# StarRocks/starrocks

Hardware: AMD Instinct MI355X
Metric: ssb_join_agg_rows_per_sec (higher is better)
Workload: dtype int64; 1 GPU; ssb_sf100_q21_star_groupby; rows_per_gpu=600000000, seed=42, parallelism=dp1-replicated-dims

## Files before the change

### starrocks_amd/csrc/gpue.hip

```cpp
#include <hip/hip_runtime.h>
#include <cassert>
#include <cstdio>
#include <cstring>
#include <cstdlib>
#include <thread>
#include <algorithm>
#include <memory>
#include <type_traits>
#include <vector>
#include "gpue.h"

static thread_local char g_err[512] = {0};

const char* gpue_last_error(void) { return g_err; }

#define HIP_CHECK(expr)                                                      \
    do {                                                                     \
        hipError_t _e = (expr);                                              \
        if (_e != hipSuccess) {                                              \
            snprintf(g_err, sizeof(g_err), "%s failed: %s (%s:%d)", #expr,   \
                     hipGetErrorString(_e), __FILE__, __LINE__);             \
            return GPUE_ERR_HIP;                                             \
        }                                                                    \
    } while (0)

#define ARG_CHECK(cond)                                                      \
    do {                                                                     \
        if (!(cond)) {                                                       \
            snprintf(g_err, sizeof(g_err), "bad argument: %s (%s:%d)",       \
                     #cond, __FILE__, __LINE__);                             \
            return GPUE_ERR_ARG;                                             \
        }                                                                    \
    } while (0)

static constexpr int BLOCK = 256;
static constexpr int WAVE = 64;
static constexpr uint64_t MAX_GRID = 2048;

static uint32_t env_cap(const char* name, uint32_t dflt) {
    const char* e = getenv(name);
    int v = e ? atoi(e) : 0;
    return v > 0 ? (uint32_t)v : dflt;
}

static inline uint32_t grid_capped(uint64_t n, uint64_t cap) {
    uint64_t b = (n + BLOCK - 1) / BLOCK;
    if (b > cap) b = cap;
    if (b == 0) b = 1;
    return (uint32_t)b;
}

static inline uint32_t grid_for(uint64_t n) {
    static uint32_t cap = 0;
    if (!cap) cap = env_cap("GPUE_GRID", MAX_GRID);
    return grid_capped(n, cap);
}

static inline uint32_t grid_stream(uint64_t n) {
    static uint32_t cap = 0;
    if (!cap) cap = env_cap("GPUE_GRID_STREAM", 256);
    return grid_capped(n, cap);
}

__device__ static inline uint32_t join_mode_count(uint32_t c, int mode) {
    switch (mode) {
    case 1: return c ? 1u : 0u;
    case 2: return c ? 0u : 1u;
    case 3: return c ? c : 1u;
    default: return c;
    }
}

struct gpue_session {
    int device;
    hipStream_t stream;
    hipEvent_t ev_start, ev_stop;
    int32_t* d_datekey = nullptr;
    void* pinned = nullptr;
    static constexpr uint64_t PINNED_BYTES = 65536;
    hipStream_t stream2 = nullptr;
    static constexpr int N_CHUNK_EVENTS = 32;
    hipEvent_t chunk_ev[N_CHUNK_EVENTS] = {};
    unsigned int* d_agg_err = nullptr;
};
#define AGG_ERR_SENTINEL 1u
#define AGG_ERR_FULL 2u

struct gpue_dbuf {
    gpue_session* s;
    void* ptr;
    uint64_t bytes;
    bool owned = true;
};

struct gpue_join_table {
    gpue_session* s = nullptr;
    int64_t min_key = 0, max_key = 0;
    uint32_t* first = nullptr;
    uint32_t* next = nullptr;
    uint32_t* bitset = nullptr;
    int64_t set_min = 0, set_max = -1;
    uint16_t* first16 = nullptr;
    uint32_t* prefilter = nullptr;
    uint32_t* prefilter2w = nullptr;
    uint32_t* prefilter2 = nullptr;
    uint2* dense_groups = nullptr;
    uint64_t bucket_size = 0;
    uint64_t row_count = 0;
    enum Kind { PAYLOAD = 0, RANGE_DIRECT = 1, BUCKET_CHAINED = 2,
                DENSE_RANGE_DIRECT = 7, BUCKET_CHAINED128 = 8,
                LINEAR_CHAINED = 3, VARCHAR = 4, BUCKET_CHAINED64 = 5 } kind = PAYLOAD;
    uint32_t log_bucket_size = 0;
    uint32_t* build_keys = nullptr;
    uint8_t* key_bytes = nullptr;
    uint32_t* key_offsets = nullptr;
    uint8_t* key_nulls = nullptr;
    uint64_t* build_keys64 = nullptr;
    ulonglong2* build_keys128 = nullptr;
};

struct JoinTableDeleter {
    void operator()(gpue_join_table* t) const { gpue_join_table_destroy(t); }
};
using JoinTableOwner = std::unique_ptr<gpue_join_table, JoinTableDeleter>;

int gpue_device_count(int* out) {
    int n = 0;
    hipError_t e = hipGetDeviceCount(&n);
    if (e != hipSuccess) n = 0;
    *out = n;
    return GPUE_OK;
}

int gpue_session_create(int device_index, gpue_session** out) {
    ARG_CHECK(out != nullptr);
    int n = 0;
    if (hipGetDeviceCount(&n) != hipSuccess || n == 0) {
        snprintf(g_err, sizeof(g_err), "no AMD GPU visible (hipGetDeviceCount)");
        return GPUE_ERR_NO_GPU;
    }
    ARG_CHECK(device_index >= 0 && device_index < n);
    HIP_CHECK(hipSetDevice(device_index));
    gpue_session* s = new gpue_session();
    s->device = device_index;
    HIP_CHECK(hipStreamCreate(&s->stream));
    HIP_CHECK(hipEventCreate(&s->ev_start));
    HIP_CHECK(hipEventCreate(&s->ev_stop));
    HIP_CHECK(hipHostMalloc(&s->pinned, gpue_session::PINNED_BYTES));
    HIP_CHECK(hipStreamCreate(&s->stream2));
    for (int i = 0; i < gpue_session::N_CHUNK_EVENTS; i++)
        HIP_CHECK(hipEventCreateWithFlags(&s->chunk_ev[i], hipEventDisableTiming));
    HIP_CHECK(hipMalloc(&s->d_agg_err, sizeof(unsigned int)));
    HIP_CHECK(hipMemset(s->d_agg_err, 0, sizeof(unsigned int)));
    *out = s;
    return GPUE_OK;
}

static int agg_err_check(gpue_session* s, const char* what) {
    unsigned int e = 0;
    HIP_CHECK(hipMemcpy(&e, s->d_agg_err, sizeof(e), hipMemcpyDeviceToHost));
    if (e == 0) return GPUE_OK;
    HIP_CHECK(hipMemset(s->d_agg_err, 0, sizeof(e)));
    snprintf(g_err, sizeof(g_err), "%s: %s%s%s", what,
             (e & AGG_ERR_SENTINEL) ? "group key 0xFFFFFFFFFFFFFFFF collides with the "
                                      "empty-slot sentinel" : "",
             (e & (AGG_ERR_SENTINEL | AGG_ERR_FULL)) == (AGG_ERR_SENTINEL | AGG_ERR_FULL)
                 ? "; " : "",
             (e & AGG_ERR_FULL) ? "hash table full (capacity < distinct keys)" : "");
    return GPUE_ERR_ARG;
}

void gpue_session_destroy(gpue_session* s) {
    if (!s) return;
    if (s->d_agg_err) (void)hipFree(s->d_agg_err);
    if (s->pinned) (void)hipHostFree(s->pinned);
    for (int i = 0; i < gpue_session::N_CHUNK_EVENTS; i++)
        if (s->chunk_ev[i]) (void)hipEventDestroy(s->chunk_ev[i]);
    if (s->stream2) (void)hipStreamDestroy(s->stream2);
    if (s->d_datekey) (void)hipFree(s->d_datekey);
    (void)hipEventDestroy(s->ev_start);
    (void)hipEventDestroy(s->ev_stop);
    (void)hipStreamDestroy(s->stream);
    delete s;
}

// ... 1203 lines not shown
            hi = max(hi, (int32_t)i);
        }
    }
    for (int off = WAVE / 2; off > 0; off >>= 1) {
        lo = min(lo, __shfl_down(lo, off, WAVE));
        hi = max(hi, __shfl_down(hi, off, WAVE));
    }
    if ((threadIdx.x & (WAVE - 1)) == 0) {
        atomicMin(lo_out, lo);
        atomicMax(hi_out, hi);
    }
}

__global__ void k_build_prefilter_split_w(const uint32_t* __restrict__ bitset,
                                          uint64_t set_interval,
                                          uint32_t* __restrict__ pf2) {
    const uint32_t M19 = (1u << 19) - 1;
    uint64_t stride = (uint64_t)gridDim.x * blockDim.x;
    for (uint64_t i = (uint64_t)blockIdx.x * blockDim.x + threadIdx.x; i < set_interval;
         i += stride) {
        if ((bitset[i >> 5] >> (i & 31)) & 1u) {
            uint32_t a = (uint32_t)i & M19;
            uint32_t b = ((uint32_t)i * 2654435761u) >> 13;
            atomicOr(&pf2[a >> 5], 1u << (a & 31));
            atomicOr(&pf2[(1u << 14) + (b >> 5)], 1u << (b & 31));
        }
    }
}

__global__ void k_build_prefilter_split(const uint32_t* __restrict__ bitset,
                                        uint64_t set_interval,
                                        uint32_t* __restrict__ pf2) {
    const uint32_t M18 = (1u << 18) - 1;
    uint64_t stride = (uint64_t)gridDim.x * blockDim.x;
    for (uint64_t i = (uint64_t)blockIdx.x * blockDim.x + threadIdx.x; i < set_interval;
         i += stride) {
        if ((bitset[i >> 5] >> (i & 31)) & 1u) {
            uint32_t a = (uint32_t)i & M18;
            uint32_t b = ((uint32_t)i * 2654435761u) >> 14;
            atomicOr(&pf2[a >> 5], 1u << (a & 31));
            atomicOr(&pf2[(1u << 13) + (b >> 5)], 1u << (b & 31));
        }
    }
}

__global__ void k_build_prefilter(const uint32_t* __restrict__ bitset, uint64_t set_interval,
                                  uint32_t* __restrict__ prefilter) {
    uint64_t stride = (uint64_t)gridDim.x * blockDim.x;
    for (uint64_t i = (uint64_t)blockIdx.x * blockDim.x + threadIdx.x; i < set_interval;
         i += stride) {
        if ((bitset[i >> 5] >> (i & 31)) & 1u) {
            uint32_t f = (uint32_t)i & ((1u << 19) - 1);
            atomicOr(&prefilter[f >> 5], 1u << (f & 31));
        }
    }
}

__global__ void k_derive_bitset(const uint32_t* __restrict__ first, uint64_t offset,
                                uint64_t interval, uint32_t* __restrict__ bitset) {
    uint64_t nwords = (interval + 31) / 32;
    uint64_t stride = (uint64_t)gridDim.x * blockDim.x;
    for (uint64_t w = (uint64_t)blockIdx.x * blockDim.x + threadIdx.x; w < nwords; w += stride) {
        uint32_t bits = 0;
        uint64_t base = w * 32;
        #pragma unroll 4
        for (int j = 0; j < 32; j++) {
            uint64_t idx = base + j;
            if (idx < interval && first[offset + idx] != 0) bits |= (1u << j);
        }
        bitset[w] = bits;
    }
}

__global__ void k_derive_u16(const uint32_t* __restrict__ first, uint64_t interval,
                             uint16_t* __restrict__ first16, uint32_t* __restrict__ overflow) {
    uint64_t stride = (uint64_t)gridDim.x * blockDim.x;
    for (uint64_t i = (uint64_t)blockIdx.x * blockDim.x + threadIdx.x; i < interval; i += stride) {
        uint32_t v = first[i];
        if (v >= 65536u) atomicOr(overflow, 1u);
        first16[i] = (uint16_t)v;
    }
}

__global__ void k_build_range_direct(const int32_t* __restrict__ keys, uint64_t row_count,
                                     int64_t min_key, uint32_t* __restrict__ first,
                                     uint32_t* __restrict__ next) {
    uint64_t stride = (uint64_t)gridDim.x * blockDim.x;
    for (uint64_t i = 1 + (uint64_t)blockIdx.x * blockDim.x + threadIdx.x; i <= row_count;
         i += stride)
        next[i] = atomicExch(&first[keys[i] - min_key], (uint32_t)i);
}

static int join_table_minmax(gpue_session* s, const int32_t* d_keys, uint64_t n,
                             int64_t* mn_out, int64_t* mx_out) {
    int32_t h_init[2] = {INT32_MAX, INT32_MIN};
    int32_t* d_mm = nullptr;
    HIP_CHECK(hipMalloc(&d_mm, 2 * sizeof(int32_t)));
    HIP_CHECK(hipMemcpyAsync(d_mm, h_init, 2 * sizeof(int32_t), hipMemcpyHostToDevice, s->stream));
    hipLaunchKernelGGL(k_minmax_i32, dim3(grid_for(n)), dim3(BLOCK), 0, s->stream,
                       d_keys, n, d_mm, d_mm + 1);
    int32_t h_mm[2];
    HIP_CHECK(hipMemcpyAsync(h_mm, d_mm, 2 * sizeof(int32_t), hipMemcpyDeviceToHost, s->stream));
    HIP_CHECK(hipStreamSynchronize(s->stream));
    (void)hipFree(d_mm);
    *mn_out = h_mm[0];
    *mx_out = h_mm[1];
    return GPUE_OK;
}

int gpue_join_build_payload_i32(gpue_session* s, gpue_dbuf* keys, gpue_dbuf* payloads,
                                uint64_t n_rows, gpue_join_table** out) {
    ARG_CHECK(s && keys && payloads && out && n_rows > 0);
    ARG_CHECK(keys->bytes >= n_rows * 4 && payloads->bytes >= n_rows * 4);
    int64_t mn, mx;
    int rc = join_table_minmax(s, (const int32_t*)keys->ptr, n_rows, &mn, &mx);
    if (rc != GPUE_OK) return rc;
    uint64_t interval = (uint64_t)(mx - mn + 1);
    ARG_CHECK(interval < (1ull << 32));
    JoinTableOwner own(new gpue_join_table());
    gpue_join_table* t = own.get();
    t->s = s; t->min_key = mn; t->max_key = mx;
    t->bucket_size = interval; t->row_count = n_rows;
    HIP_CHECK(hipMalloc(&t->first, interval * sizeof(uint32_t)));
    HIP_CHECK(hipMemsetAsync(t->first, 0, interval * sizeof(uint32_t), s->stream));
    hipLaunchKernelGGL(k_build_payload, dim3(grid_for(n_rows)), dim3(BLOCK), 0, s->stream,
                       (const int32_t*)keys->ptr, (const uint32_t*)payloads->ptr, n_rows,
                       mn, t->first);
    HIP_CHECK(hipGetLastError());
    int32_t h_bounds[2] = {INT32_MAX, INT32_MIN};
    DevScratch tmp;
    int32_t* d_bounds = nullptr;
    HIP_CHECK(tmp.alloc(&d_bounds, 2 * sizeof(int32_t)));
    HIP_CHECK(hipMemcpyAsync(d_bounds, h_bounds, sizeof(h_bounds), hipMemcpyHostToDevice,
                             s->stream));
    hipLaunchKernelGGL(k_set_bounds, dim3(grid_for(interval)), dim3(BLOCK), 0, s->stream,
                       t->first, interval, d_bounds, d_bounds + 1);
    HIP_CHECK(hipMemcpyAsync(h_bounds, d_bounds, sizeof(h_bounds), hipMemcpyDeviceToHost,
                             s->stream));
    HIP_CHECK(hipStreamSynchronize(s->stream));
    uint64_t set_off, set_interval;
    if (h_bounds[0] > h_bounds[1]) {
        t->set_min = mn;
        t->set_max = mn;
        set_off = 0;
        set_interval = 1;
    } else {
        t->set_min = mn + h_bounds[0];
        t->set_max = mn + h_bounds[1];
        set_off = (uint64_t)h_bounds[0];
        set_interval = (uint64_t)(h_bounds[1] - h_bounds[0] + 1);
    }
    uint64_t nwords = (set_interval + 31) / 32;
    HIP_CHECK(hipMalloc(&t->bitset, nwords * sizeof(uint32_t)));
    hipLaunchKernelGGL(k_derive_bitset, dim3(grid_for(nwords)), dim3(BLOCK), 0, s->stream,
                       t->first, set_off, set_interval, t->bitset);
    HIP_CHECK(hipMalloc(&t->prefilter, (1u << 19) / 8));
    HIP_CHECK(hipMemsetAsync(t->prefilter, 0, (1u << 19) / 8, s->stream));
    hipLaunchKernelGGL(k_build_prefilter, dim3(grid_for(set_interval)), dim3(BLOCK), 0,
                       s->stream, t->bitset, set_interval, t->prefilter);
    HIP_CHECK(hipMalloc(&t->prefilter2, (1u << 19) / 8));
    HIP_CHECK(hipMemsetAsync(t->prefilter2, 0, (1u << 19) / 8, s->stream));
    hipLaunchKernelGGL(k_build_prefilter_split, dim3(grid_for(set_interval)), dim3(BLOCK),
                       0, s->stream, t->bitset, set_interval, t->prefilter2);
    HIP_CHECK(hipMalloc(&t->prefilter2w, (1u << 20) / 8));
    HIP_CHECK(hipMemsetAsync(t->prefilter2w, 0, (1u << 20) / 8, s->stream));
    hipLaunchKernelGGL(k_build_prefilter_split_w, dim3(grid_for(set_interval)), dim3(BLOCK),
                       0, s->stream, t->bitset, set_interval, t->prefilter2w);
    uint32_t* d_ovf = nullptr;
    HIP_CHECK(tmp.alloc(&d_ovf, sizeof(uint32_t)));
    HIP_CHECK(hipMemsetAsync(d_ovf, 0, sizeof(uint32_t), s->stream));
    HIP_CHECK(hipMalloc(&t->first16, interval * sizeof(uint16_t)));
    hipLaunchKernelGGL(k_derive_u16, dim3(grid_for(interval)), dim3(BLOCK), 0, s->stream,
                       t->first, interval, t->first16, d_ovf);
    uint32_t ovf = 0;
    HIP_CHECK(hipMemcpyAsync(&ovf, d_ovf, sizeof(uint32_t), hipMemcpyDeviceToHost, s->stream));
    HIP_CHECK(hipStreamSynchronize(s->stream));
    if (ovf) { (void)hipFree(t->first16); t->first16 = nullptr; }
    *out = own.release();
    return GPUE_OK;
}

int gpue_join_build_range_direct_i32(gpue_session* s, gpue_dbuf* keys, uint64_t row_count,
                                     gpue_join_table** out) {
    ARG_CHECK(s && keys && out && row_count > 0);
    ARG_CHECK(keys->bytes >= (row_count + 1) * 4);
    int64_t mn, mx;
    int rc = join_table_minmax(s, (const int32_t*)keys->ptr + 1, row_count, &mn, &mx);
    if (rc != GPUE_OK) return rc;
    uint64_t interval = (uint64_t)(mx - mn + 1);
    ARG_CHECK(interval < (1ull << 32));
    JoinTableOwner own(new gpue_join_table());
    gpue_join_table* t = own.get();
    t->s = s; t->min_key = mn; t->max_key = mx;
    t->bucket_size = interval; t->row_count = row_count;
    t->kind = gpue_join_table::RANGE_DIRECT;
    HIP_CHECK(hipMalloc(&t->first, interval * sizeof(uint32_t)));
    HIP_CHECK(hipMalloc(&t->next, (row_count + 1) * sizeof(uint32_t)));
    HIP_CHECK(hipMemsetAsync(t->first, 0, interval * sizeof(uint32_t), s->stream));
    HIP_CHECK(hipMemsetAsync(t->next, 0, (row_count + 1) * sizeof(uint32_t), s->stream));
    hipLaunchKernelGGL(k_build_range_direct, dim3(grid_for(row_count)), dim3(BLOCK), 0,
                       s->stream, (const int32_t*)keys->ptr, row_count, mn, t->first, t->next);
    HIP_CHECK(hipGetLastError());
    *out = own.release();
    return GPUE_OK;
}

void gpue_join_table_destroy(gpue_join_table* t) {
    if (!t) return;
    if (t->first) (void)hipFree(t->first);
    if (t->next) (void)hipFree(t->next);
    if (t->bitset) (void)hipFree(t->bitset);
    if (t->first16) (void)hipFree(t->first16);
    if (t->prefilter) (void)hipFree(t->prefilter);
    if (t->prefilter2) (void)hipFree(t->prefilter2);
    if (t->prefilter2w) (void)hipFree(t->prefilter2w);
    if (t->dense_groups) (void)hipFree(t->dense_groups);
    if (t->build_keys) (void)hipFree(t->build_keys);
    if (t->key_bytes) (void)hipFree(t->key_bytes);
    if (t->key_offsets) (void)hipFree(t->key_offsets);
    if (t->key_nulls) (void)hipFree(t->key_nulls);
    if (t->build_keys64) (void)hipFree(t->build_keys64);
    if (t->build_keys128) (void)hipFree(t->build_keys128);
    delete t;
}

int gpue_join_table_minmax(gpue_join_table* t, int64_t* min_out, int64_t* max_out) {
    ARG_CHECK(t && min_out && max_out);
    *min_out = t->min_key;
    *max_out = t->max_key;
    return GPUE_OK;
}

int gpue_join_table_first_d2h(gpue_join_table* t, uint32_t* dst, uint64_t n_entries) {
    ARG_CHECK(t && dst && n_entries <= t->bucket_size);
    HIP_CHECK(hipMemcpy(dst, t->first, n_entries * sizeof(uint32_t), hipMemcpyDeviceToHost));
    return GPUE_OK;
}

__device__ static inline uint32_t join_hash_u32(uint32_t v, uint32_t num_log_buckets) {
    v ^= v >> (32 - num_log_buckets);
    return (v * 2654435761u) >> (32 - num_log_buckets);
}

__device__ static inline uint32_t join_hash_u64_dev(uint64_t v, uint32_t num_log_buckets) {
    v ^= v >> (64 - num_log_buckets);
    return (uint32_t)((v * 11400714819323198485ull) >> (64 - num_log_buckets));
}

struct HashU32 {
    uint32_t log_bucket_size;
    static HashU32 of(const gpue_join_table* t) { return {t->log_bucket_size}; }
    __device__ uint32_t operator()(uint32_t k) const {
        return join_hash_u32(k, log_bucket_size);
    }
};
struct HashU64 {
    uint32_t log_bucket_size;
    static HashU64 of(const gpue_join_table* t) { return {t->log_bucket_size}; }
    __device__ uint32_t operator()(uint64_t k) const {
        return join_hash_u64_dev(k, log_bucket_size);
    }
};

template <class K, class H, bool NULLS>
__global__ void k_build_bucket_chained(const K* __restrict__ keys,
                                       const uint8_t* __restrict__ is_nulls,
                                       uint64_t row_count, H hash,
                                       uint32_t* __restrict__ first,
                                       uint32_t* __restrict__ next) {
    uint64_t stride = (uint64_t)gridDim.x * blockDim.x;
    for (uint64_t i = 1 + (uint64_t)blockIdx.x * blockDim.x + threadIdx.x; i <= row_count;
         i += stride) {
        if (NULLS && is_nulls[i]) continue;
        const K k = keys[i];
        next[i] = atomicExch(&first[hash(k)], (uint32_t)i);
    }
}

__global__ void k_pack_keys_2xi32(const int32_t* __restrict__ a,
                                  const int32_t* __restrict__ b, uint64_t n,
                                  uint64_t* __restrict__ out) {
    uint64_t stride = (uint64_t)gridDim.x * blockDim.x;
    for (uint64_t i = (uint64_t)blockIdx.x * blockDim.x + threadIdx.x; i < n; i += stride)
        out[i] = (uint64_t)(uint32_t)a[i] | ((uint64_t)(uint32_t)b[i] << 32);
}

extern "C" int gpue_pack_keys_2xi32(gpue_session* s, gpue_dbuf* a, gpue_dbuf* b, uint64_t n,
                                    gpue_dbuf* out);
int gpue_pack_keys_2xi32(gpue_session* s, gpue_dbuf* a, gpue_dbuf* b, uint64_t n,
                         gpue_dbuf* out) {
    ARG_CHECK(s && a && b && out && out->bytes >= n * 8);
    hipLaunchKernelGGL(k_pack_keys_2xi32, dim3(grid_stream(n)), dim3(BLOCK), 0, s->stream,
                       (const int32_t*)a->ptr, (const int32_t*)b->ptr, n,
                       (uint64_t*)out->ptr);
    HIP_CHECK(hipGetLastError());
// ... 2926 lines not shown
        uint32_t ia = (in ? idx : 0u) & ((1u << 18) - 1);
        uint32_t ib = ((in ? idx : 0u) * 2654435761u) >> 14;
        bool maybe = in & (pfa[ia >> 5] >> (ia & 31)) & (pfb[ib >> 5] >> (ib & 31)) & 1u;
        uint64_t m = __ballot(maybe);
        if (m) {
            if (maybe) q1[wid][n1 + __popcll(m & below)] = make_int2(key, (int32_t)row);
            n1 += __popcll(m);
            if (n1 >= 64) drain1(64);
        }
    };
    auto ld4nt = [&](const int4* p, uint64_t i) {
        const uint64_t* q = (const uint64_t*)(p + i);
        uint64_t lo = __builtin_nontemporal_load(q);
        uint64_t hi = __builtin_nontemporal_load(q + 1);
        int4 v;
        v.x = (int32_t)lo; v.y = (int32_t)(lo >> 32);
        v.z = (int32_t)hi; v.w = (int32_t)(hi >> 32);
        return v;
    };
    uint64_t base = (uint64_t)blockIdx.x * blockDim.x + (uint64_t)wid * WAVE;
    uint64_t i = base + lane;
    if constexpr (PREFETCH) {
        bool more = base + stride + WAVE <= n4;
        int4 pa = make_int4(0, 0, 0, 0), pb_ = pa;
        if (more) {
            pa = ld4nt(pk4, i);
            pb_ = ld4nt(pk4, i + stride);
        }
        while (more) {
            const uint64_t ci = i, ci2 = i + stride;
            base += 2 * stride;
            i += 2 * stride;
            more = base + stride + WAVE <= n4;
            int4 na = pa, nb = pb_;
            if (more) {
                na = ld4nt(pk4, i);
                nb = ld4nt(pk4, i + stride);
            }
            #pragma unroll
            for (int j = 0; j < 4; j++) push((&pa.x)[j], (uint32_t)(ci * 4 + j), true);
            #pragma unroll
            for (int j = 0; j < 4; j++) push((&pb_.x)[j], (uint32_t)(ci2 * 4 + j), true);
            pa = na;
            pb_ = nb;
        }
    } else {
        for (; base + stride + WAVE <= n4; base += 2 * stride, i += 2 * stride) {
            int4 pa = ld4nt(pk4, i);
            uint64_t i2 = i + stride;
            int4 pb_ = ld4nt(pk4, i2);
            #pragma unroll
            for (int j = 0; j < 4; j++) push((&pa.x)[j], (uint32_t)(i * 4 + j), true);
            #pragma unroll
            for (int j = 0; j < 4; j++) push((&pb_.x)[j], (uint32_t)(i2 * 4 + j), true);
        }
    }
    for (; base < n4; base += stride, i += stride) {
        bool inb = i < n4;
        int4 p4 = inb ? pk4[i] : make_int4(0, 0, 0, 0);
        #pragma unroll
        for (int j = 0; j < 4; j++) push((&p4.x)[j], (uint32_t)(i * 4 + j), inb);
    }
    if (n1 > 0) drain1(n1);
    if constexpr (B > 0) {
        if (n2 > 0) drain2(n2);
        if (n3 > 0) drain3(n3);
    }
    uint64_t tid = (uint64_t)blockIdx.x * blockDim.x + threadIdx.x;
    for (uint64_t r = n4 * 4 + tid; r < n; r += stride) {
        uint32_t idx = (uint32_t)(pk[r] - psmin);
        if (idx >= psint) continue;
        uint32_t brand1 = pfirst[pk[r] - 1];
        if (!brand1) continue;
        uint32_t sidx = (uint32_t)(sk[r] - ssmin);
        if (sidx >= ssint || !((sbits[sidx >> 5] >> (sidx & 31)) & 1u)) continue;
        uint32_t year1 = dfirst[od[r] - dmin];
        atomicAdd(&g[(year1 - 1) * 1000 + (brand1 - 1)], (unsigned long long)(int64_t)rv[r]);
    }
    __syncthreads();
    for (int j = threadIdx.x; j < NG_Q21; j += blockDim.x)
        if (g[j] != 0) atomicAdd(&group_sums[j], g[j]);
}

__global__ void k_q21_pass_payload(const int32_t* __restrict__ pk, uint64_t n,
                                   const uint32_t* __restrict__ pbits, int64_t psmin,
                                   uint64_t psint, const uint16_t* __restrict__ pfirst,
                                   uint16_t* __restrict__ brand_out) {
    const uint64_t n4 = n / 4;
    const int4* __restrict__ pk4 = (const int4*)pk;
    uint64_t stride = (uint64_t)gridDim.x * blockDim.x;
    uint64_t i = (uint64_t)blockIdx.x * blockDim.x + threadIdx.x;
    for (; i + stride < n4; i += 2 * stride) {
        int4 pa = pk4[i];
        int4 pb_ = pk4[i + stride];
        ushort4 oa, ob;
        #pragma unroll
        for (int j = 0; j < 4; j++) {
            uint32_t idx = (uint32_t)((&pa.x)[j] - psmin);
            bool in = idx < psint;
            uint32_t cidx = in ? idx : 0u;
            bool pass = in & ((pbits[cidx >> 5] >> (cidx & 31)) & 1u);
            (&oa.x)[j] = pass ? pfirst[(&pa.x)[j] - 1] : (uint16_t)0;
        }
        #pragma unroll
        for (int j = 0; j < 4; j++) {
            uint32_t idx = (uint32_t)((&pb_.x)[j] - psmin);
            bool in = idx < psint;
            uint32_t cidx = in ? idx : 0u;
            bool pass = in & ((pbits[cidx >> 5] >> (cidx & 31)) & 1u);
            (&ob.x)[j] = pass ? pfirst[(&pb_.x)[j] - 1] : (uint16_t)0;
        }
        ((ushort4*)brand_out)[i] = oa;
        ((ushort4*)brand_out)[i + stride] = ob;
    }
    for (; i < n4; i += stride) {
        int4 p4 = pk4[i];
        ushort4 o;
        #pragma unroll
        for (int j = 0; j < 4; j++) {
            uint32_t idx = (uint32_t)((&p4.x)[j] - psmin);
            bool in = idx < psint;
            uint32_t cidx = in ? idx : 0u;
            bool pass = in & ((pbits[cidx >> 5] >> (cidx & 31)) & 1u);
            (&o.x)[j] = pass ? pfirst[(&p4.x)[j] - 1] : (uint16_t)0;
        }
        ((ushort4*)brand_out)[i] = o;
    }
    uint64_t tid = (uint64_t)blockIdx.x * blockDim.x + threadIdx.x;
    for (uint64_t r = n4 * 4 + tid; r < n; r += stride) {
        uint32_t idx = (uint32_t)(pk[r] - psmin);
        bool in = idx < psint;
        uint32_t cidx = in ? idx : 0u;
        bool pass = in & ((pbits[cidx >> 5] >> (cidx & 31)) & 1u);
        brand_out[r] = pass ? pfirst[pk[r] - 1] : (uint16_t)0;
    }
}

__global__ __launch_bounds__(BLOCK_Q21) void
k_q21_phase2(const uint16_t* __restrict__ brand, const int32_t* __restrict__ sk,
             const int32_t* __restrict__ od, const int32_t* __restrict__ rv, uint64_t n,
             const uint32_t* __restrict__ sbits, int64_t ssmin, uint64_t ssint,
             const uint16_t* __restrict__ dfirst, int64_t dmin,
             unsigned long long* __restrict__ group_sums) {
    __shared__ unsigned long long g[NG_Q21];
    for (int j = threadIdx.x; j < NG_Q21; j += blockDim.x) g[j] = 0;
    __syncthreads();
    const uint64_t n4 = n / 4;
    const ushort4* __restrict__ br4 = (const ushort4*)brand;
    const int4* __restrict__ sk4 = (const int4*)sk;
    const int4* __restrict__ od4 = (const int4*)od;
    const int4* __restrict__ rv4 = (const int4*)rv;
    uint64_t stride = (uint64_t)gridDim.x * blockDim.x;
    for (uint64_t i = (uint64_t)blockIdx.x * blockDim.x + threadIdx.x; i < n4; i += stride) {
        ushort4 b4 = br4[i];
        int4 s4 = sk4[i];
        int4 o4 = od4[i];
        int4 r4 = rv4[i];
        #pragma unroll
        for (int j = 0; j < 4; j++) {
            uint16_t brand1 = (&b4.x)[j];
            if (brand1 == 0) continue;
            uint32_t sidx = (uint32_t)((&s4.x)[j] - ssmin);
            if (sidx >= ssint || !((sbits[sidx >> 5] >> (sidx & 31)) & 1u)) continue;
            uint32_t year1 = dfirst[(&o4.x)[j] - dmin];
            atomicAdd(&g[(year1 - 1) * 1000 + (brand1 - 1)],
                      (unsigned long long)(int64_t)(&r4.x)[j]);
        }
    }
    uint64_t tid = (uint64_t)blockIdx.x * blockDim.x + threadIdx.x;
    for (uint64_t r = n4 * 4 + tid; r < n; r += stride) {
        uint16_t brand1 = brand[r];
        if (brand1 == 0) continue;
        uint32_t sidx = (uint32_t)(sk[r] - ssmin);
        if (sidx >= ssint || !((sbits[sidx >> 5] >> (sidx & 31)) & 1u)) continue;
        uint32_t year1 = dfirst[od[r] - dmin];
        atomicAdd(&g[(year1 - 1) * 1000 + (brand1 - 1)], (unsigned long long)(int64_t)rv[r]);
    }
    __syncthreads();
    for (int j = threadIdx.x; j < NG_Q21; j += blockDim.x)
        if (g[j] != 0) atomicAdd(&group_sums[j], g[j]);
}

extern "C" int gpue_q21_star_agg_pipe(gpue_session* s, gpue_join_table* parts,
                                      gpue_join_table* supps, gpue_join_table* dates,
                                      gpue_dbuf* pk, gpue_dbuf* sk, gpue_dbuf* od,
                                      gpue_dbuf* rv, uint64_t n, gpue_dbuf* brand_scratch,
                                      gpue_dbuf* group_sums, int n_chunks);
int gpue_q21_star_agg_pipe(gpue_session* s, gpue_join_table* parts, gpue_join_table* supps,
                           gpue_join_table* dates, gpue_dbuf* pk, gpue_dbuf* sk,
                           gpue_dbuf* od, gpue_dbuf* rv, uint64_t n,
                           gpue_dbuf* brand_scratch, gpue_dbuf* group_sums, int n_chunks) {
    ARG_CHECK(s && parts && supps && dates && pk && sk && od && rv && brand_scratch &&
              group_sums);
    ARG_CHECK(parts->first16 && parts->bitset && supps->bitset && dates->first16);
    ARG_CHECK(brand_scratch->bytes >= n * 2);
    ARG_CHECK(n_chunks >= 1 && n_chunks <= gpue_session::N_CHUNK_EVENTS);
    HIP_CHECK(hipMemsetAsync(group_sums->ptr, 0, NG_Q21 * sizeof(int64_t), s->stream));
    uint64_t per = (n + (uint64_t)n_chunks - 1) / (uint64_t)n_chunks;
    uint64_t chunk = (per + 3) & ~3ull;
    for (int c = 0; c < n_chunks; c++) {
        uint64_t lo = (uint64_t)c * chunk;
        if (lo >= n) break;
        uint64_t len = min(chunk, n - lo);
        hipLaunchKernelGGL(k_q21_pass_payload, dim3(grid_for(len)), dim3(BLOCK), 0,
                           s->stream2, (const int32_t*)pk->ptr + lo, len, parts->bitset,
                           parts->set_min, (uint64_t)(parts->set_max - parts->set_min + 1),
                           parts->first16, (uint16_t*)brand_scratch->ptr + lo);
        HIP_CHECK(hipEventRecord(s->chunk_ev[c], s->stream2));
        HIP_CHECK(hipStreamWaitEvent(s->stream, s->chunk_ev[c], 0));
        hipLaunchKernelGGL(k_q21_phase2, dim3(env_cap("GPUE_GRID_WIDE", 512)),
                           dim3(BLOCK_Q21), 0, s->stream,
                           (const uint16_t*)brand_scratch->ptr + lo,
                           (const int32_t*)sk->ptr + lo, (const int32_t*)od->ptr + lo,
                           (const int32_t*)rv->ptr + lo, len, supps->bitset,
                           supps->set_min, (uint64_t)(supps->set_max - supps->set_min + 1),
                           dates->first16, dates->min_key,
                           (unsigned long long*)group_sums->ptr);
    }
    HIP_CHECK(hipGetLastError());
    return GPUE_OK;
}

static bool q21_glob() {
    static int v = -1;
    if (v < 0) {
        const char* e = getenv("GPUE_Q21_GLOB");
        v = (e && atoi(e)) ? 1 : 0;
    }
    return v == 1;
}

static bool q21_pf() {
    static int v = -1;
    if (v < 0) {
        const char* e = getenv("GPUE_Q21_PF");
        v = (e && !atoi(e)) ? 0 : 1;
    }
    return v == 1;
}

extern "C" int gpue_q21_star_agg_async(gpue_session* s, gpue_join_table* parts,
                                       gpue_join_table* supps, gpue_join_table* dates,
                                       gpue_dbuf* pk, gpue_dbuf* sk, gpue_dbuf* od,
                                       gpue_dbuf* rv, uint64_t n, gpue_dbuf* group_sums);
int gpue_q21_star_agg_async(gpue_session* s, gpue_join_table* parts, gpue_join_table* supps,
                            gpue_join_table* dates, gpue_dbuf* pk, gpue_dbuf* sk,
                            gpue_dbuf* od, gpue_dbuf* rv, uint64_t n, gpue_dbuf* group_sums) {
    ARG_CHECK(s && parts && supps && dates && pk && sk && od && rv && group_sums);
    ARG_CHECK(group_sums->bytes >= NG_Q21 * sizeof(int64_t));
    ARG_CHECK(parts->min_key == 1 && supps->min_key == 1);
    ARG_CHECK(parts->first16 && supps->first16 && dates->first16);
    HIP_CHECK(hipMemsetAsync(group_sums->ptr, 0, NG_Q21 * sizeof(int64_t), s->stream));
    if (q21_pf() && parts->prefilter) {
        const char* e = getenv("GPUE_Q21_PF");
        int mode = e ? atoi(e) : 8;
        const char* nt = getenv("GPUE_Q21_PF_NT");
        bool use_nt = !nt || atoi(nt);
        int def_grid = mode == 2 ? 512 : 256;
        int tpb = env_cap("GPUE_Q21_PF_TPB", BLOCK_Q21);
        auto launch = [&](auto kern, int grid) {
            hipLaunchKernelGGL(kern, dim3(env_cap("GPUE_GRID_PF", grid)),
                               dim3(tpb), 0, s->stream, (const int32_t*)pk->ptr,
                               (const int32_t*)sk->ptr, (const int32_t*)od->ptr,
                               (const int32_t*)rv->ptr, n, parts->prefilter, parts->set_min,
                               (uint64_t)(parts->set_max - parts->set_min + 1),
                               parts->first16, supps->bitset, supps->set_min,
                               (uint64_t)(supps->set_max - supps->set_min + 1),
                               dates->first16, dates->min_key,
                               (unsigned long long*)group_sums->ptr);
        };
        ARG_CHECK((mode != 7 && mode != 8) || n <= UINT32_MAX);
        if (mode == 8) {
            auto launch8 = [&](auto kern) {
                hipLaunchKernelGGL(kern, dim3(env_cap("GPUE_GRID_PF", def_grid)),
                                   dim3(tpb), 0, s->stream, (const int32_t*)pk->ptr,
                                   (const int32_t*)sk->ptr, (const int32_t*)od->ptr,
                                   (const int32_t*)rv->ptr, n, parts->prefilter2,
                                   parts->set_min,
                                   (uint64_t)(parts->set_max - parts->set_min + 1),
                                   parts->first16, supps->bitset, supps->set_min,
                                   (uint64_t)(supps->set_max - supps->set_min + 1),
                                   dates->first16, dates->min_key,
                                   (unsigned long long*)group_sums->ptr);
            };
            int var = (int)env_cap("GPUE_Q21_PF8_VAR", 11);
            ARG_CHECK(var == 10 || var == 1 || var == 11 || var == 12);
            if (var == 10) launch8(k_q21_star_agg_pfq4<true, 0>);
            else if (var == 1) launch8(k_q21_star_agg_pfq4<false, 1>);
            else if (var == 11) launch8(k_q21_star_agg_pfq4<true, 1>);
            else launch8(k_q21_star_agg_pfq4<true, 2>);
        }
        else if (mode == 7) {
            hipLaunchKernelGGL(k_q21_star_agg_pfq3, dim3(env_cap("GPUE_GRID_PF", def_grid)),
                               dim3(tpb), 0, s->stream, (const int32_t*)pk->ptr,
                               (const int32_t*)sk->ptr, (const int32_t*)od->ptr,
                               (const int32_t*)rv->ptr, n, parts->prefilter2,
                               parts->set_min,
                               (uint64_t)(parts->set_max - parts->set_min + 1),
                               parts->first16, supps->bitset, supps->set_min,
                               (uint64_t)(supps->set_max - supps->set_min + 1),
                               dates->first16, dates->min_key,
                               (unsigned long long*)group_sums->ptr);
        }
        else if (mode == 6) {
            hipLaunchKernelGGL(k_q21_star_agg_pfq2, dim3(env_cap("GPUE_GRID_PF", def_grid)),
                               dim3(tpb), 0, s->stream, (const int32_t*)pk->ptr,
                               (const int32_t*)sk->ptr, (const int32_t*)od->ptr,
                               (const int32_t*)rv->ptr, n, parts->prefilter2,
                               parts->set_min,
                               (uint64_t)(parts->set_max - parts->set_min + 1),
                               parts->first16, supps->bitset, supps->set_min,
                               (uint64_t)(supps->set_max - supps->set_min + 1),
                               dates->first16, dates->min_key,
                               (unsigned long long*)group_sums->ptr);
        }
        else if (mode == 4) launch(k_q21_star_agg_pfq, def_grid);
        else if (mode == 2 && use_nt) launch(k_q21_star_agg_pf<false, true>, def_grid);
        else if (mode == 2) launch(k_q21_star_agg_pf<false, false>, def_grid);
        else if (use_nt) launch(k_q21_star_agg_pf<true, true>, def_grid);
        else launch(k_q21_star_agg_pf<true, false>, def_grid);
        HIP_CHECK(hipGetLastError());
        return GPUE_OK;
    }
    if (q21_glob()) {
        hipLaunchKernelGGL(k_q21_star_agg_glob, dim3(grid_stream(n)), dim3(BLOCK), 0,
                           s->stream, (const int32_t*)pk->ptr, (const int32_t*)sk->ptr,
                           (const int32_t*)od->ptr, (const int32_t*)rv->ptr, n,
                           parts->bitset, parts->set_min,
                           (uint64_t)(parts->set_max - parts->set_min + 1), parts->first16,
                           supps->bitset, supps->set_min,
                           (uint64_t)(supps->set_max - supps->set_min + 1), dates->first16,
                           dates->min_key, (unsigned long long*)group_sums->ptr);
    } else
    hipLaunchKernelGGL(k_q21_star_agg, dim3(env_cap("GPUE_GRID_WIDE", 512)), dim3(BLOCK_Q21), 0, s->stream,
                       (const int32_t*)pk->ptr, (const int32_t*)sk->ptr,
                       (const int32_t*)od->ptr, (const int32_t*)rv->ptr, n,
                       parts->bitset, parts->set_min,
                       (uint64_t)(parts->set_max - parts->set_min + 1), parts->first16,
                       supps->bitset, supps->set_min,
                       (uint64_t)(supps->set_max - supps->set_min + 1), dates->first16,
                       dates->min_key, (unsigned long long*)group_sums->ptr);
    HIP_CHECK(hipGetLastError());
    return GPUE_OK;
}

int gpue_q21_star_agg(gpue_session* s, gpue_join_table* parts, gpue_join_table* supps,
                      gpue_join_table* dates, gpue_dbuf* pk, gpue_dbuf* sk, gpue_dbuf* od,
                      gpue_dbuf* rv, uint64_t n, int64_t* group_sums_out) {
    ARG_CHECK(s && parts && supps && dates && pk && sk && od && rv && group_sums_out);
    ARG_CHECK(pk->bytes >= n * 4 && sk->bytes >= n * 4 && od->bytes >= n * 4 && rv->bytes >= n * 4);
    ARG_CHECK(parts->min_key == 1 && supps->min_key == 1);
    ARG_CHECK(parts->first16 && supps->first16 && dates->first16);
    unsigned long long* d_g = nullptr;
    HIP_CHECK(hipMalloc(&d_g, NG_Q21 * sizeof(unsigned long long)));
    gpue_dbuf tmp{s, d_g, NG_Q21 * sizeof(unsigned long long), false};
// ... 4254 lines not shown
```

Baseline: 590.3 billion rows/s.

## Compact part payloads to dense ranks and add pfq5 Q2.1 star-agg kernel

At build time, the distinct brand payloads of the part table are ranked into a dense table of at most 64 entries, and a remapped first16c array is stored alongside the originals. A new kernel, k_q21_star_agg_pfq5, uses these ranks. It keeps a much smaller shared-memory group accumulator (7×64 instead of the full group space) and stages survivors through wave-local queues for the part, supplier and date probes, with a K-way burst of nontemporal key loads. The goal is to shrink shared-memory footprint and atomic contention and to raise occupancy. The cost is an extra host round-trip at table build, and the path only applies when there are no more than 64 distinct payloads and pay_max is at most 1000.

Result: faster. 604.0 billion rows/s, median of 6 (+2.3%).

```diff
diff --git a/starrocks_amd/csrc/gpue.hip b/starrocks_amd/csrc/gpue.hip
--- a/starrocks_amd/csrc/gpue.hip
+++ b/starrocks_amd/csrc/gpue.hip
@@ -93,6 +93,8 @@
     bool owned = true;
 };
 
+static constexpr uint32_t NBC = 64;
+
 struct gpue_join_table {
     gpue_session* s = nullptr;
     int64_t min_key = 0, max_key = 0;
@@ -101,6 +103,10 @@
     uint32_t* bitset = nullptr;
     int64_t set_min = 0, set_max = -1;
     uint16_t* first16 = nullptr;
+    uint16_t* first16c = nullptr;
+    uint16_t* pay_vals = nullptr;
+    uint32_t n_pay = 0;
+    uint32_t pay_max = 0;
     uint32_t* prefilter = nullptr;
     uint32_t* prefilter2w = nullptr;
     uint32_t* prefilter2 = nullptr;
@@ -1470,6 +1476,67 @@
     }
 }
 
+__global__ void k_mark_payloads(const uint16_t* __restrict__ first16, uint64_t interval,
+                                uint32_t* __restrict__ marks) {
+    __shared__ uint32_t m[2048];
+    for (uint32_t w = threadIdx.x; w < 2048; w += blockDim.x) m[w] = 0;
+    __syncthreads();
+    uint64_t stride = (uint64_t)gridDim.x * blockDim.x;
+    for (uint64_t i = (uint64_t)blockIdx.x * blockDim.x + threadIdx.x; i < interval; i += stride) {
+        uint32_t v = first16[i];
+        if (v && !((m[v >> 5] >> (v & 31)) & 1u)) atomicOr(&m[v >> 5], 1u << (v & 31));
+    }
+    __syncthreads();
+    for (uint32_t w = threadIdx.x; w < 2048; w += blockDim.x)
+        if (m[w]) atomicOr(&marks[w], m[w]);
+}
+
+__global__ void k_rank_u16(const uint16_t* __restrict__ first16, uint64_t interval,
+                           const uint8_t* __restrict__ rank1, uint16_t* __restrict__ first16c) {
+    uint64_t stride = (uint64_t)gridDim.x * blockDim.x;
+    for (uint64_t i = (uint64_t)blockIdx.x * blockDim.x + threadIdx.x; i < interval; i += stride)
+        first16c[i] = rank1[first16[i]];
+}
+
+static int join_table_rank_payloads(gpue_session* s, gpue_join_table* t, uint64_t interval) {
+    DevScratch tmp;
+    uint32_t* d_marks = nullptr;
+    HIP_CHECK(tmp.alloc(&d_marks, 2048 * sizeof(uint32_t)));
+    HIP_CHECK(hipMemsetAsync(d_marks, 0, 2048 * sizeof(uint32_t), s->stream));
+    hipLaunchKernelGGL(k_mark_payloads, dim3(grid_for(interval)), dim3(BLOCK), 0, s->stream,
+                       t->first16, interval, d_marks);
+    std::vector<uint32_t> marks(2048);
+    HIP_CHECK(hipMemcpyAsync(marks.data(), d_marks, 2048 * sizeof(uint32_t),
+                             hipMemcpyDeviceToHost, s->stream));
+    HIP_CHECK(hipStreamSynchronize(s->stream));
+    std::vector<uint8_t> rank1(65536, 0);
+    uint16_t vals[NBC];
+    uint32_t n_pay = 0;
+    for (uint32_t v = 1; v < 65536; v++)
+        if ((marks[v >> 5] >> (v & 31)) & 1u) {
+            if (n_pay == NBC) return GPUE_OK;
+            vals[n_pay++] = (uint16_t)v;
+            rank1[v] = (uint8_t)n_pay;
+        }
+    uint8_t* d_rank1 = nullptr;
+    HIP_CHECK(tmp.alloc(&d_rank1, rank1.size()));
+    HIP_CHECK(hipMemcpyAsync(d_rank1, rank1.data(), rank1.size(), hipMemcpyHostToDevice,
+                             s->stream));
+    HIP_CHECK(hipMalloc(&t->pay_vals, NBC * sizeof(uint16_t)));
+    HIP_CHECK(hipMemsetAsync(t->pay_vals, 0, NBC * sizeof(uint16_t), s->stream));
+    if (n_pay)
+        HIP_CHECK(hipMemcpyAsync(t->pay_vals, vals, n_pay * sizeof(uint16_t),
+                                 hipMemcpyHostToDevice, s->stream));
+    HIP_CHECK(hipMalloc(&t->first16c, interval * sizeof(uint16_t)));
+    hipLaunchKernelGGL(k_rank_u16, dim3(grid_for(interval)), dim3(BLOCK), 0, s->stream,
+                       t->first16, interval, d_rank1, t->first16c);
+    HIP_CHECK(hipGetLastError());
+    HIP_CHECK(hipStreamSynchronize(s->stream));
+    t->n_pay = n_pay;
+    t->pay_max = n_pay ? vals[n_pay - 1] : 0;
+    return GPUE_OK;
+}
+
 __global__ void k_build_range_direct(const int32_t* __restrict__ keys, uint64_t row_count,
                                      int64_t min_key, uint32_t* __restrict__ first,
                                      uint32_t* __restrict__ next) {
@@ -1564,6 +1631,10 @@
     HIP_CHECK(hipMemcpyAsync(&ovf, d_ovf, sizeof(uint32_t), hipMemcpyDeviceToHost, s->stream));
     HIP_CHECK(hipStreamSynchronize(s->stream));
     if (ovf) { (void)hipFree(t->first16); t->first16 = nullptr; }
+    if (t->first16) {
+        rc = join_table_rank_payloads(s, t, interval);
+        if (rc != GPUE_OK) return rc;
+    }
     *out = own.release();
     return GPUE_OK;
 }
@@ -1599,6 +1670,8 @@
     if (t->next) (void)hipFree(t->next);
     if (t->bitset) (void)hipFree(t->bitset);
     if (t->first16) (void)hipFree(t->first16);
+    if (t->first16c) (void)hipFree(t->first16c);
+    if (t->pay_vals) (void)hipFree(t->pay_vals);
     if (t->prefilter) (void)hipFree(t->prefilter);
     if (t->prefilter2) (void)hipFree(t->prefilter2);
     if (t->prefilter2w) (void)hipFree(t->prefilter2w);
@@ -4691,6 +4764,157 @@
         if (g[j] != 0) atomicAdd(&group_sums[j], g[j]);
 }
 
+template <int FA, int Q1CAP, int K>
+__global__ __launch_bounds__(BLOCK_Q21) void
+k_q21_star_agg_pfq5(const int32_t* __restrict__ pk, const int32_t* __restrict__ sk,
+                    const int32_t* __restrict__ od, const int32_t* __restrict__ rv,
+                    uint64_t n, const uint32_t* __restrict__ folda,
+                    const uint32_t* __restrict__ foldb, int64_t psmin, uint64_t psint,
+                    const uint16_t* __restrict__ pfirstc,
+                    const uint16_t* __restrict__ pay_vals, uint32_t n_pay,
+                    const uint32_t* __restrict__ sbits, int64_t ssmin, uint64_t ssint,
+                    const uint16_t* __restrict__ dfirst, int64_t dmin,
+                    unsigned long long* __restrict__ group_sums) {
+    static_assert(FA == 18 || FA == 19, "fold A is one of the table's two masked folds");
+    static_assert(Q1CAP == 128 || Q1CAP >= 320, "see the fill bounds above");
+    static_assert(K >= 1 && (K == 1 || Q1CAP >= 320), "a burst needs the per-quad guard");
+    constexpr bool PERKEY = Q1CAP == 128;
+    constexpr int QS = 126 + 64;
+    constexpr uint32_t WA = 1u << (FA - 5);
+    __shared__ uint32_t pfa[WA];
+    __shared__ uint32_t pfb[1 << 13];
+    __shared__ unsigned long long g[7 * NBC];
+    __shared__ int2 q1[BLOCK_Q21 / WAVE][Q1CAP];
+    __shared__ uint32_t qrow[BLOCK_Q21 / WAVE][QS];
+    __shared__ uint16_t qbr[BLOCK_Q21 / WAVE][QS];
+    for (uint32_t w = threadIdx.x; w < WA; w += blockDim.x) pfa[w] = folda[w];
+    for (uint32_t w = threadIdx.x; w < (1u << 13); w += blockDim.x) pfb[w] = foldb[w];
+    for (uint32_t j = threadIdx.x; j < 7 * NBC; j += blockDim.x) g[j] = 0;
+    __syncthreads();
+    const int wid = threadIdx.x / WAVE;
+    const uint32_t lane = threadIdx.x & (WAVE - 1);
+    const uint64_t below = (1ull << lane) - 1;
+    uint32_t n1 = 0, n2 = 0, n3 = 0;
+    const uint64_t n4 = n / 4;
+    const int4* __restrict__ pk4 = (const int4*)pk;
+    uint64_t stride = (uint64_t)gridDim.x * blockDim.x;
+    auto drain3 = [&](uint32_t cnt) {
+        bool act = lane < cnt;
+        uint32_t slot = QS - 1 - (n3 - cnt + lane);
+        uint32_t r = act ? qrow[wid][slot] : 0u;
+        uint32_t b = act ? qbr[wid][slot] : 0u;
+        n3 -= cnt;
+        if (act) {
+            int32_t o = od[r];
+            int32_t v = rv[r];
+            uint32_t y = dfirst[o - dmin];
+            atomicAdd(&g[(y - 1) * NBC + (b - 1)], (unsigned long long)(int64_t)v);
+        }
+    };
+    auto drain2 = [&](uint32_t cnt) {
+        bool act = lane < cnt;
+        uint32_t r = act ? qrow[wid][n2 - cnt + lane] : 0u;
+        uint32_t b = act ? qbr[wid][n2 - cnt + lane] : 0u;
+        n2 -= cnt;
+        bool pass = false;
+        if (act) {
+            uint32_t sidx = (uint32_t)(sk[r] - ssmin);
+            pass = sidx < ssint && ((sbits[sidx >> 5] >> (sidx & 31)) & 1u);
+        }
+        uint64_t m = __ballot(pass);
+        if (m) {
+            if (pass) {
+                uint32_t slot = QS - 1 - (n3 + __popcll(m & below));
+                qrow[wid][slot] = r;
+                qbr[wid][slot] = (uint16_t)b;
+            }
+            n3 += __popcll(m);
+            if (n3 >= 64) drain3(64);
+        }
+    };
+    auto drain1 = [&](uint32_t cnt) {
+        bool act = lane < cnt;
+        int2 e = act ? q1[wid][n1 - cnt + lane] : make_int2(1, 0);
+        n1 -= cnt;
+        uint32_t rank1 = act ? pfirstc[e.x - 1] : 0u;
+        uint64_t m = __ballot(rank1 != 0);
+        if (m) {
+            if (rank1) {
+                uint32_t slot = n2 + __popcll(m & below);
+                qrow[wid][slot] = (uint32_t)e.y;
+                qbr[wid][slot] = (uint16_t)rank1;
+            }
+            n2 += __popcll(m);
+            if (n2 >= 64) drain2(64);
+        }
+    };
+    auto push = [&](int32_t key, uint32_t row, bool inb) {
+        uint32_t idx = (uint32_t)(key - psmin);
+        bool in = inb & (idx < psint);
+        uint32_t ia = (in ? idx : 0u) & ((1u << FA) - 1);
+        uint32_t ib = ((in ? idx : 0u) * 2654435761u) >> 14;
+        bool maybe = in & (pfa[ia >> 5] >> (ia & 31)) & (pfb[ib >> 5] >> (ib & 31)) & 1u;
+        uint64_t m = __ballot(maybe);
+        if (m) {
+            if (maybe) q1[wid][n1 + __popcll(m & below)] = make_int2(key, (int32_t)row);
+            n1 += __popcll(m);
+            if constexpr (PERKEY)
+                if (n1 >= 64) drain1(64);
+        }
+    };
+    auto quad = [&](int4 p, uint64_t qi, bool inb) {
+        if constexpr (!PERKEY)
+            while (n1 + 256 > Q1CAP) drain1(64);
+        #pragma unroll
+        for (int j = 0; j < 4; j++) push((&p.x)[j], (uint32_t)(qi * 4 + j), inb);
+    };
+    auto ld4nt = [&](const int4* p, uint64_t i) {
+        const uint64_t* q = (const uint64_t*)(p + i);
+        uint64_t lo = __builtin_nontemporal_load(q);
+        uint64_t hi = __builtin_nontemporal_load(q + 1);
+        int4 v;
+        v.x = (int32_t)lo; v.y = (int32_t)(lo >> 32);
+        v.z = (int32_t)hi; v.w = (int32_t)(hi >> 32);
+        return v;
+    };
+    uint64_t base = (uint64_t)blockIdx.x * blockDim.x + (uint64_t)wid * WAVE;
+    uint64_t i = base + lane;
+    for (; base + (K - 1) * stride + WAVE <= n4; base += K * stride, i += K * stride) {
+        int4 p[K];
+        #pragma unroll
+        for (int k = 0; k < K; k++) p[k] = ld4nt(pk4, i + k * stride);
+        #pragma unroll
+        for (int k = 0; k < K; k++) quad(p[k], i + k * stride, true);
+        while (n1 >= 64) drain1(64);
+    }
+    for (; base < n4; base += stride, i += stride) {
+        bool inb = i < n4;
+        int4 p4 = inb ? pk4[i] : make_int4(0, 0, 0, 0);
+        quad(p4, i, inb);
+        while (n1 >= 64) drain1(64);
+    }
+    if (n1 > 0) drain1(n1);
+    if (n2 > 0) drain2(n2);
+    if (n3 > 0) drain3(n3);
+    uint64_t tid = (uint64_t)blockIdx.x * blockDim.x + threadIdx.x;
+    for (uint64_t r = n4 * 4 + tid; r < n; r += stride) {
+        uint32_t idx = (uint32_t)(pk[r] - psmin);
+        if (idx >= psint) continue;
+        uint32_t rank1 = pfirstc[pk[r] - 1];
+        if (!rank1) continue;
+        uint32_t sidx = (uint32_t)(sk[r] - ssmin);
+        if (sidx >= ssint || !((sbits[sidx >> 5] >> (sidx & 31)) & 1u)) continue;
+        uint32_t year1 = dfirst[od[r] - dmin];
+        atomicAdd(&g[(year1 - 1) * NBC + (rank1 - 1)], (unsigned long long)(int64_t)rv[r]);
+    }
+    __syncthreads();
+    for (uint32_t j = threadIdx.x; j < 7 * n_pay; j += blockDim.x) {
+        uint32_t y = j / n_pay, r = j - y * n_pay;
+        unsigned long long v = g[y * NBC + r];
+        if (v != 0) atomicAdd(&group_sums[y * 1000 + pay_vals[r] - 1], v);
+    }
+}
+
 __global__ void k_q21_pass_payload(const int32_t* __restrict__ pk, uint64_t n,
                                    const uint32_t* __restrict__ pbits, int64_t psmin,
                                    uint64_t psint, const uint16_t* __restrict__ pfirst,
@@ -4848,6 +5072,8 @@
     return v == 1;
 }
 
+static constexpr int Q21_PF9_DEFAULT_VAR = 4;
+
 extern "C" int gpue_q21_star_agg_async(gpue_session* s, gpue_join_table* parts,
                                        gpue_join_table* supps, gpue_join_table* dates,
                                        gpue_dbuf* pk, gpue_dbuf* sk, gpue_dbuf* od,
@@ -4862,7 +5088,9 @@
     HIP_CHECK(hipMemsetAsync(group_sums->ptr, 0, NG_Q21 * sizeof(int64_t), s->stream));
     if (q21_pf() && parts->prefilter) {
         const char* e = getenv("GPUE_Q21_PF");
-        int mode = e ? atoi(e) : 8;
+        const bool compact_ok = parts->first16c && parts->prefilter2 && parts->prefilter2w &&
+                                parts->pay_max <= 1000 && n <= UINT32_MAX;
+        int mode = e ? atoi(e) : (compact_ok && Q21_PF9_DEFAULT_VAR > 0) ? 9 : 8;
         const char* nt = getenv("GPUE_Q21_PF_NT");
         bool use_nt = !nt || atoi(nt);
         int def_grid = mode == 2 ? 512 : 256;
@@ -4879,7 +5107,30 @@
                                (unsigned long long*)group_sums->ptr);
         };
         ARG_CHECK((mode != 7 && mode != 8) || n <= UINT32_MAX);
-        if (mode == 8) {
+        if (mode == 9) {
+            ARG_CHECK(compact_ok);
+            int var = (int)env_cap("GPUE_Q21_PF9_VAR",
+                                   Q21_PF9_DEFAULT_VAR > 0 ? Q21_PF9_DEFAULT_VAR : 1);
+            ARG_CHECK(var >= 1 && var <= 4);
+            auto launch9 = [&](auto kern, const uint32_t* folda) {
+                hipLaunchKernelGGL(kern, dim3(env_cap("GPUE_GRID_PF", def_grid)),
+                                   dim3(tpb), 0, s->stream, (const int32_t*)pk->ptr,
+                                   (const int32_t*)sk->ptr, (const int32_t*)od->ptr,
+                                   (const int32_t*)rv->ptr, n, folda,
+                                   parts->prefilter2 + (1u << 13), parts->set_min,
+                                   (uint64_t)(parts->set_max - parts->set_min + 1),
+                                   parts->first16c, parts->pay_vals, parts->n_pay,
+                                   supps->bitset, supps->set_min,
+                                   (uint64_t)(supps->set_max - supps->set_min + 1),
+                                   dates->first16, dates->min_key,
+                                   (unsigned long long*)group_sums->ptr);
+            };
+            if (var == 1) launch9(k_q21_star_agg_pfq5<18, 128, 1>, parts->prefilter2);
+            else if (var == 2) launch9(k_q21_star_agg_pfq5<19, 128, 1>, parts->prefilter2w);
+            else if (var == 3) launch9(k_q21_star_agg_pfq5<18, 384, 4>, parts->prefilter2);
+            else launch9(k_q21_star_agg_pfq5<19, 320, 4>, parts->prefilter2w);
+        }
+        else if (mode == 8) {
             auto launch8 = [&](auto kern) {
                 hipLaunchKernelGGL(kern, dim3(env_cap("GPUE_GRID_PF", def_grid)),
                                    dim3(tpb), 0, s->stream, (const int32_t*)pk->ptr,
```
